# alexmillerdb/two_tower_recommender_model

Hardware: AMD Instinct MI355X
Metric: training pairs/sec at batch 8192 (per GPU) (higher is better)
Workload: dtype fp32; 1 GPU; northstar: 100M items x 50M users, emb_dim 128, towers [128, 64], single-hot uniform ids; global_batch=8192, per_gpu_batch=8192, emb_dim=128, tower_dtype=bf16 (MFMA, fp32 acc), parallelism=single-gpu hipgraph

## Files before the change

### two_tower_recommender_model_amd/csrc/tower.hip

```cpp
#include <vector>

#include "tt_common.h"
#include "dedup.h"
#include "shard.h"

namespace tt {

typedef __attribute__((ext_vector_type(8))) __bf16 bf16x8;
typedef __attribute__((ext_vector_type(4))) float f32x4;
typedef __attribute__((ext_vector_type(4))) __bf16 bf16x4;

constexpr int TR = 32;
constexpr int MAXW = 128;
constexpr int XCH = 128;
constexpr int LSTR = MAXW + 8;
constexpr int FSTR = MAXW + 4;
constexpr int MAXL = 4;

__device__ __forceinline__ int64_t strip_at(int64_t f, int64_t m, int64_t nf) {
  return (((m >> 5) * nf + f) << 5) + (m & 31);
}

struct TowerArgs {
  tt_tower_shape_t s;
// ... 1028 lines not shown
__host__ __device__ __forceinline__ int rk_swz(int row) {
  return (row & 3) | (((row & 1) | (((row >> 3) & 1) << 1)) << 2);
}
__host__ __device__ __forceinline__ int rk_off(int row, int col) {
  return row * 256 + (((col >> 3) ^ rk_swz(row)) << 4) + ((col & 7) << 1);
}
__device__ __forceinline__ int rk_perm(int mt, int rho) {
  return 32 * (mt >> 1) + 8 * (rho >> 2) + 4 * (mt & 1) + (rho & 3);
}
__device__ __forceinline__ bf16x8 rk_afwd(const char* img, int mt, int s, int rho, int q) {
  return *reinterpret_cast<const bf16x8*>(img + rk_off(rk_perm(mt, rho), 32 * s + 8 * q));
}
__device__ __forceinline__ bf16x8 rk_abwd(const char* img, int mt, int s, int lane) {
  const int q = lane >> 4, qq = (lane >> 2) & 3, p = lane & 3;
  const int row = 32 * s + 8 * q + qq;
  const int col = 32 * (mt >> 1) + 8 * p + 4 * (mt & 1);
  const bf16x4 lo = __builtin_amdgcn_ds_read_tr16_b64_v4bf16((lds_bf16x4*)(img + rk_off(row, col)));
  const bf16x4 hi = __builtin_amdgcn_ds_read_tr16_b64_v4bf16((lds_bf16x4*)(img + rk_off(row + 4, col)));
  return __builtin_shufflevector(lo, hi, 0, 1, 2, 3, 4, 5, 6, 7);
}
__device__ __forceinline__ bf16x8 rk_pack(const f32x4& a, const f32x4& b) {
  bf16x8 v;
#pragma unroll
  for (int j = 0; j < 4; ++j) {
    v[j] = (__bf16)a[j];
    v[4 + j] = (__bf16)b[j];
  }
  return v;
}
template <int MT, int S, bool BWD>
__device__ __forceinline__ void rk_gemm(f32x4 (&acc)[8], const char* img, const bf16x8 (&b)[4], int lane) {
  const int n = lane & 15, q = lane >> 4;
  bf16x8 fa[2][MT];
#pragma unroll
  for (int mt = 0; mt < MT; ++mt) {
    acc[mt] = (f32x4)(0.f);
    fa[0][mt] = BWD ? rk_abwd(img, mt, 0, lane) : rk_afwd(img, mt, 0, n, q);
  }
#pragma unroll
  for (int s = 0; s < S; ++s) {
    if (s + 1 < S) {
#pragma unroll
      for (int mt = 0; mt < MT; ++mt)
        fa[(s + 1) & 1][mt] = BWD ? rk_abwd(img, mt, s + 1, lane) : rk_afwd(img, mt, s + 1, n, q);
    }
    __builtin_amdgcn_sched_barrier(0);
#pragma unroll
    for (int mt = 0; mt < MT; ++mt)
      acc[mt] = __builtin_amdgcn_mfma_f32_16x16x32_bf16(fa[s & 1][mt], b[s], acc[mt], 0, 0, 0);
    __builtin_amdgcn_sched_barrier(0);
  }
}
template <int X>
__device__ __forceinline__ float rk_xor(float v) {
  if constexpr (X == 1) return dpp_f<0xB1>(v);
  if constexpr (X == 2) return dpp_f<0x4E>(v);
  if constexpr (X == 4) return dpp_f<0x1B>(dpp_f<0x141>(v));
  return dpp_f<0x128>(v);
}
template <int X, int H>
__device__ __forceinline__ void rk_halve(float* v, int n) {
  const bool up = (n & X) != 0;
#pragma unroll
  for (int i = 0; i < H; ++i) {
    const float keep = up ? v[H + i] : v[i], send = up ? v[i] : v[H + i];
    v[i] = keep + rk_xor<X>(send);
  }
}
template <int NV>
__device__ __forceinline__ void rk_colsum(float (&v)[NV], int n) {
  static_assert(NV == 32 || NV == 16, "column sum of 32 or 16 values per lane");
  rk_halve<8, NV / 2>(v, n);
  rk_halve<4, NV / 4>(v, n);
  rk_halve<2, NV / 8>(v, n);
  rk_halve<1, NV / 16>(v, n);
}
template <int NS>
__device__ __forceinline__ void rk_strip(const bf16x8 (&v)[4], __bf16* row, int q) {
#pragma unroll
  for (int s = 0; s < NS; ++s) *reinterpret_cast<bf16x8*>(row + 32 * s + 8 * q) = v[s];
}


__device__ __forceinline__ char* px_row(const tt_peer_direct_t& x, int64_t row, int64_t row_bytes) {
  char* base = reinterpret_cast<char*>(x.row0[0]);
  int64_t f0 = 0;
#pragma unroll
  for (int q = 1; q < TT_PEER_MAXW; ++q) {
    if (q < x.W && row >= x.first_row[q]) {
      base = reinterpret_cast<char*>(x.row0[q]);
      f0 = x.first_row[q];
    }
  }
  return base + (row - f0) * row_bytes;
}
__device__ __forceinline__ bool px_copy_unit(const tt_peer_direct_t& x, int64_t u, const uint4*& src, uint4*& dst) {
  int64_t pre = 0;
  bool hit = false;
#pragma unroll
  for (int q = 0; q < TT_PEER_MAXW; ++q) {
    const int64_t n = q < x.W ? x.copy_len[q] >> 4 : 0;
    if (!hit && u >= pre && u < pre + n) {
      src = reinterpret_cast<const uint4*>(x.copy_src[q]) + (u - pre);
      dst = reinterpret_cast<uint4*>(x.copy_dst[q]) + (u - pre);
      hit = true;
    }
    pre += n;
  }
  return hit;
}
__device__ __forceinline__ int64_t px_copy_units(const tt_peer_direct_t& x) {
  int64_t n = 0;
#pragma unroll
  for (int q = 0; q < TT_PEER_MAXW; ++q) n += q < x.W ? x.copy_len[q] >> 4 : 0;
  return n;
}

struct RkRaw {
  uint32_t lo, hi;
};
__device__ __forceinline__ RkRaw rk_raw(const void* p, bool wide, int64_t i) {
  RkRaw r;
  if (wide) {
    const uint2 v = reinterpret_cast<const uint2*>(p)[i];
    r.lo = v.x;
    r.hi = v.y;
  } else {
    r.lo = reinterpret_cast<const uint32_t*>(p)[i];
    r.hi = 0u;
  }
  return r;
}
__device__ __forceinline__ int64_t rk_id(RkRaw r, bool wide) {
  return wide ? (int64_t)(((uint64_t)r.hi << 32) | r.lo) : (int64_t)(int32_t)r.lo;
}
__device__ __forceinline__ float rk_label(RkRaw r, int dt) {
  if (dt == TT_I32) return (float)(int32_t)r.lo;
  if (dt == TT_I64) return (float)(int64_t)(((uint64_t)r.hi << 32) | r.lo);
  return __uint_as_float(r.lo);
}
#if TT_EXPERIMENTS
#define RK_STAMP(k) \
  do { if (a.stamps && lane == 0) a.stamps[8192 + ((int64_t)blockIdx.x * 16 + (k)) * 9 + wid] = (int64_t)__builtin_amdgcn_s_memrealtime(); } while (0)
#define RK_STAMP2(k) \
  do { if (a.stamps && lane == 0) a.stamps[8192 + ((int64_t)blockIdx.x * 16 + (k)) * 9 + 4 + wid] = (int64_t)__builtin_amdgcn_s_memrealtime(); } while (0)
#define RK_STAMP_IMG(k) \
  do { if (a.stamps && lane == 0) a.stamps[8192 + ((int64_t)blockIdx.x * 16 + (k)) * 9 + 8] = (int64_t)__builtin_amdgcn_s_memrealtime(); } while (0)
#else
#define RK_STAMP(k) do { } while (0)
#define RK_STAMP2(k) do { } while (0)
#define RK_STAMP_IMG(k) do { } while (0)
#endif

struct UpdateArgs {
  float* params;
  float* exp_avg;
  float* exp_avg_sq;
  const float* slab;
  const float* dbpart;
  int64_t P;
  int S;
  int nwg;
  int nseg;
  int64_t seg_off[2 * 2 * MAXL + 1];
  int32_t seg_t[2 * 2 * MAXL], seg_l[2 * 2 * MAXL], seg_isw[2 * 2 * MAXL], seg_n[2 * 2 * MAXL], seg_k[2 * 2 * MAXL];
  int64_t seg_wc[2 * 2 * MAXL];
  __bf16* wb;
  __bf16* wtb;
  __bf16* wbf;
  __bf16* wtbf;
  int skip_plain;
  float lr, beta1, beta2, eps, wd;
  int64_t* step_state;
  int do_adam;
  float* grads_out;
  const float* grads_in;
  const float* adam_pre;
  int out_copies;
  int64_t out_stride;
  int64_t out_off[16];
  float out_scale;
  int in_srcs;
  int64_t in_stride;
  char* wimg;
  PxWait wt;
#if TT_EXPERIMENTS
  int64_t* stamps;
#endif
};
#if TT_EXPERIMENTS
#define T3_STAMP(k) \
  do { if (a.stamps && threadIdx.x == 0 && bid < 512) a.stamps[(int64_t)bid * 4 + (k)] = (int64_t)__builtin_amdgcn_s_memrealtime(); } while (0)
#else
#define T3_STAMP(k) do { } while (0)
#endif

struct T3Seg {
  int64_t soff = 0, swc = 0;
  int sisw = 0, sk = 1, sn = 1, st_ = 0, sl_ = 0;
};
__device__ __forceinline__ T3Seg t3_seg(const UpdateArgs& a, int64_t i) {
  T3Seg g;
#pragma unroll
  for (int q = 0; q < 2 * 2 * MAXL; ++q) {
    if (q < a.nseg && i >= a.seg_off[q]) {
      g.soff = a.seg_off[q];
      g.sisw = a.seg_isw[q];
      g.sk = a.seg_k[q];
      g.sn = a.seg_n[q];
      g.swc = a.seg_wc[q];
      g.st_ = a.seg_t[q];
      g.sl_ = a.seg_l[q];
    }
  }
  return g;
}

__device__ __forceinline__ void t3_apply(const UpdateArgs& a, int64_t i, const T3Seg& sg, float p, float m,
                                         float v0, float g, float step_size, float bc2_sqrt, bool adam) {
#pragma clang fp contract(off)
  const int64_t e = i - sg.soff;
  if (a.grads_out) {
    if (a.out_copies <= 1) {
      a.grads_out[i] = g;
    } else {
      const float gs = g * a.out_scale;
      for (int q = 0; q < a.out_copies; ++q) a.grads_out[a.out_off[q] + i] = gs;
    }
  }
  if (adam) {
    if (a.wd != 0.f) g = g + a.wd * p;
    m = m + (1.f - a.beta1) * (g - m);
    const float v = v0 * a.beta2 + (1.f - a.beta2) * g * g;
    const float denom = sqrtf(v) / bc2_sqrt + a.eps;
    p = p + (-step_size) * m / denom;
    a.exp_avg[i] = m;
    a.exp_avg_sq[i] = v;
    a.params[i] = p;
  }
  if (sg.sisw) {
    const int K = sg.sk, N = sg.sn;
    const int64_t n = e / K, k = e - n * K;
    if (!a.skip_plain) {
      a.wb[sg.swc + e] = (__bf16)p;
      a.wtb[sg.swc + k * N + n] = (__bf16)p;
    }
    a.wbf[sg.swc + frag_off((int)n, (int)k, K)] = (__bf16)p;
    a.wtbf[sg.swc + frag_off((int)k, (int)n, N)] = (__bf16)p;
    if (a.wimg)
      *reinterpret_cast<__bf16*>(a.wimg + sg.st_ * RK_IMG_T + sg.sl_ * (RK_W0 * 256) + rk_off((int)n, (int)k)) = (__bf16)p;
  }
}

template <bool UPD, bool IDX, int IN, bool POOL = false>
__device__ __forceinline__ void tower_rows_body(const TowerArgs& a) {
  static_assert(IN == 128 || IN == 64, "row-owned T1: inputs of 128 or 64");
  static_assert(!POOL || (!UPD && !IDX), "pooled input: the plain T1 only");
  constexpr int NI = IN / 32;
  constexpr int MTI = IN / 16;
  __shared__ __attribute__((aligned(16))) char wimg[RK_IMG];
  __shared__ __attribute__((aligned(16))) float xo[2][2][16 * 64];
  __shared__ float bsum[2][RK_W0 + RK_W1];
  __shared__ float lrow[TR];
  __shared__ __attribute__((aligned(16))) float xr[4][16 * IN];
  const int lane = threadIdx.x & 63, wid = __builtin_amdgcn_readfirstlane(threadIdx.x >> 6);
  typedef __attribute__((address_space(3))) void lds_void;
  typedef __attribute__((address_space(1))) void glb_void;
  if (wid == 4) {
    RK_STAMP_IMG(0);
    if (!TDBG(16)) {
#pragma unroll
      for (int k = 0; k < RK_IMG / 1024; ++k)
        __builtin_amdgcn_global_load_lds((glb_void*)(a.wimg + k * 1024 + lane * 16), (lds_void*)(wimg + k * 1024), 16, 0, 0);
    }
    RK_STAMP_IMG(1);
    __builtin_amdgcn_s_waitcnt(0x0F70);
    RK_STAMP_IMG(2);
    __syncthreads();
    RK_STAMP_IMG(3);
    __syncthreads();
    __syncthreads();
    return;
  }
  const int t = wid >> 1, h = wid & 1, q = lane >> 4, n = lane & 15;
  const int tile = xcd_remap((int)blockIdx.x, (int)gridDim.x);
  const int64_t B = a.B, m0 = (int64_t)tile * TR, m = m0 + 16 * h + n;
  const bool live = m < B;
  RK_STAMP(0);
  const bool wide = a.gid_dtype == TT_I64;
  const int64_t mc = live ? m : 0;
  RkRaw id_raw{0u, 0u}, pout_raw{0u, 0u};
  if (IDX) {
    id_raw.lo = (uint32_t)(t ? a.gpos[1] : a.gpos[0])[mc];
    pout_raw.lo = a.gpos_out[0] ? (uint32_t)(t ? a.gpos_out[1] : a.gpos_out[0])[mc] : id_raw.lo;
  } else if (!POOL) {
    id_raw = rk_raw(t ? a.gcol[1] : a.gcol[0], wide, mc);
  }
  int32_t cl = -1;
  if (UPD) cl = a.dd.claim[live ? t * B + m : 0];
  const RkRaw lab_raw = rk_raw(a.labels, a.label_dtype == TT_I64, mc);
  f32x4 b0v[8], b1v[4];
  auto load_biases = [&]() {
    const float* b0p = a.params + a.boff[t][0];
    const float* b1p = a.params + a.boff[t][1];
#pragma unroll
    for (int mt = 0; mt < 8; ++mt) b0v[mt] = *reinterpret_cast<const f32x4*>(b0p + 32 * (mt >> 1) + 8 * q + 4 * (mt & 1));
#pragma unroll
    for (int mt = 0; mt < 4; ++mt) b1v[mt] = *reinterpret_cast<const f32x4*>(b1p + 32 * (mt >> 1) + 8 * q + 4 * (mt & 1));
  };
  load_biases();
  __builtin_amdgcn_sched_barrier(0);
  uint4 cpv = make_uint4(0u, 0u, 0u, 0u);
  uint4* cpd = nullptr;
  int64_t cp_per = 0, cp_end = 0;
  if constexpr (IDX) {
    if (a.xd.W) {
      const int64_t tot = px_copy_units(a.xd);
      cp_per = (tot + gridDim.x - 1) / gridDim.x;
      cp_end = min(tot, ((int64_t)blockIdx.x + 1) * cp_per);
      const int64_t u = (int64_t)blockIdx.x * cp_per + threadIdx.x;
      const uint4* cps;
      if (u < cp_end && px_copy_unit(a.xd, u, cps, cpd)) cpv = *cps;
      else cpd = nullptr;
    }
  }
  int64_t r;
  if (POOL) {
    r = live ? m : -1;
  } else if (IDX) {
    r = live ? (int64_t)(int32_t)id_raw.lo : -1;
  } else {
    const int64_t id = live ? rk_id(id_raw, wide) : 0;
    r = id != 0 ? py_mod64(id, t ? a.gmod[1] : a.gmod[0]) : -1;
  }
  const float* tab = POOL ? a.pooled + a.s.in_col[t] : (t ? a.gtab[1] : a.gtab[0]);
  const int64_t rstride = POOL ? a.ldp : IN;
  float* xw = xr[wid];
  constexpr int CPR = IDX ? IN / 8 : IN / 4;
  constexpr int RPI = 64 / CPR;
  if (IDX) {
    const int rr0 = lane / CPR, pc = lane % CPR;
    const char* src0 = reinterpret_cast<const char*>(t ? a.gsrc[1] : a.gsrc[0]);
#pragma unroll
    for (int i = 0; i < 16 / RPI; ++i) {
      const int row = RPI * i + rr0;
      const int64_t rid = __shfl((long long)r, row, 64);
      const char* src = src0 + (rid >= 0 ? rid : 0) * (IN * 2) + 16 * (pc ^ (row & (CPR - 1)));
      __builtin_amdgcn_global_load_lds((glb_void*)src, (lds_void*)(reinterpret_cast<char*>(xw) + i * 1024), 16, 0, 0);
    }
  } else {
    const int rr0 = lane / CPR, pc = lane % CPR;
#pragma unroll
    for (int i = 0; i < 16 / RPI; ++i) {
      const int row = RPI * i + rr0;
      const int64_t rid = __shfl((long long)r, row, 64);
      const float* src = tab + (rid >= 0 ? rid : 0) * rstride + 4 * (pc ^ row);
      if (!TDBG(32))
        __builtin_amdgcn_global_load_lds((glb_void*)src, (lds_void*)(xw + i * 256), 16, 0, 0);
    }
  }
  __builtin_amdgcn_sched_barrier(0);
  DdPend pend;
  pend.key = DD_EMPTY;
  const int32_t li = (int32_t)(t * B + m);
  if (!UPD && a.dd_on && q == 0 && live) {
    const uint64_t key = r >= 0 ? (((uint64_t)(t ? a.dd_table[1] : a.dd_table[0]) << DD_TABLE_SHIFT) | (uint64_t)r)
                                : DD_EMPTY;
// ... 689 lines not shown
  }
  for (; m + 32 <= me; m += 32) {
    const int64_t o = m + q * 8;
    const bf16x8 fa0 = *reinterpret_cast<const bf16x8*>(z0 + zo(o));
    const bf16x8 fa1 = *reinterpret_cast<const bf16x8*>(z1 + zo(o));
    const bf16x8 fb0 = *reinterpret_cast<const bf16x8*>(a0 + ao(o));
    const bf16x8 fb1 = *reinterpret_cast<const bf16x8*>(a1 + ao(o));
    acc[0][0] = __builtin_amdgcn_mfma_f32_16x16x32_bf16(fa0, fb0, acc[0][0], 0, 0, 0);
    acc[0][1] = __builtin_amdgcn_mfma_f32_16x16x32_bf16(fa0, fb1, acc[0][1], 0, 0, 0);
    acc[1][0] = __builtin_amdgcn_mfma_f32_16x16x32_bf16(fa1, fb0, acc[1][0], 0, 0, 0);
    acc[1][1] = __builtin_amdgcn_mfma_f32_16x16x32_bf16(fa1, fb1, acc[1][1], 0, 0, 0);
  }
  if (m < me) {
    bf16x8 fa0, fa1, fb0, fb1;
    for (int j = 0; j < 8; ++j) {
      const int64_t mm = m + q * 8 + j;
      const bool ok = mm < me;
      fa0[j] = ok ? z0[zo(mm)] : (__bf16)0.f;
      fa1[j] = ok ? z1[zo(mm)] : (__bf16)0.f;
      fb0[j] = ok ? a0[ao(mm)] : (__bf16)0.f;
      fb1[j] = ok ? a1[ao(mm)] : (__bf16)0.f;
    }
    acc[0][0] = __builtin_amdgcn_mfma_f32_16x16x32_bf16(fa0, fb0, acc[0][0], 0, 0, 0);
    acc[0][1] = __builtin_amdgcn_mfma_f32_16x16x32_bf16(fa0, fb1, acc[0][1], 0, 0, 0);
    acc[1][0] = __builtin_amdgcn_mfma_f32_16x16x32_bf16(fa1, fb0, acc[1][0], 0, 0, 0);
    acc[1][1] = __builtin_amdgcn_mfma_f32_16x16x32_bf16(fa1, fb1, acc[1][1], 0, 0, 0);
  }
  if (wid > 0) {
#pragma unroll
    for (int i = 0; i < 2; ++i)
#pragma unroll
      for (int j = 0; j < 2; ++j)
#pragma unroll
        for (int rr = 0; rr < 4; ++rr) red[wid - 1][((i * 2 + j) * 4 + rr) * 64 + lane] = acc[i][j][rr];
  }
  __syncthreads();
  if (wid > 0) return;
#pragma unroll
  for (int w = 0; w < 3; ++w)
#pragma unroll
    for (int i = 0; i < 2; ++i)
#pragma unroll
      for (int j = 0; j < 2; ++j)
#pragma unroll
        for (int rr = 0; rr < 4; ++rr) acc[i][j][rr] += red[w][((i * 2 + j) * 4 + rr) * 64 + lane];
  const int K = a.K[tl.t][tl.l];
  float* dst = a.slab + (int64_t)s * a.P + a.woff[tl.t][tl.l];
  for (int i = 0; i < 2; ++i)
    for (int j = 0; j < 2; ++j)
      for (int rr = 0; rr < 4; ++rr) {
        const int n = tl.n0 + i * 16 + q * 4 + rr;
        const int k = tl.k0 + j * 16 + r;
        dst[(int64_t)n * K + k] = acc[i][j][rr];
      }
}

__global__ void __launch_bounds__(256) tower_wgrad_kernel(WgradArgs a, const WgradTile* __restrict__ tiles) {
  __shared__ __attribute__((aligned(16))) char smem[T2_SMEM];
  if ((int)blockIdx.x < a.n_res)
    dd_resolve_block(a.dd, (int)blockIdx.x, a.n_res);
  else
    wgrad_block(a, tiles, (int)blockIdx.x - a.n_res, smem);
}

__global__ void __launch_bounds__(256) tower_wgrad_dedup_kernel(WgradArgs a, const WgradTile* __restrict__ tiles,
                                                                DdUpdateArgs d, int n_t2) {
  __shared__ __attribute__((aligned(16))) char smem[T2_SMEM];
  if ((int)blockIdx.x < n_t2)
    wgrad_block(a, tiles, (int)blockIdx.x, smem);
  else
    dd_update_block(d, (int)blockIdx.x - n_t2, smem);
}

struct InsertArgs {
  const void* col[2];
  int64_t mod[2];
  int32_t tab[2];
  int id_dtype;
  int64_t B;
  DedupWs dd;
  int xcd_wpt;
};
__device__ __forceinline__ int64_t ins_lookup(const InsertArgs& ins, int blk, int tid) {
  if (ins.xcd_wpt <= 0) return (int64_t)blk * 256 + tid;
  const int c = blk & 7, j = blk >> 3;
  const int t = j / ins.xcd_wpt, qi = j - t * ins.xcd_wpt;
  const int64_t b = (int64_t)c * (ins.B / 256) + 8 * qi + (tid >> 5);
  return (int64_t)t * ins.B + 32 * b + (tid & 31);
}

__device__ __forceinline__ void insert_next_block(const InsertArgs& ins, int blk) {
  const int lane = threadIdx.x & 63;
  const int64_t grp = (int64_t)blk * 4 + (threadIdx.x >> 6);
  const int64_t i = grp * 64 + lane;
  DdPend p;
  p.key = DD_EMPTY;
  if (i < 2 * ins.B) {
    const int t = i >= ins.B;
    const int64_t m = i - (t ? ins.B : 0);
    const int64_t id = load_id(t ? ins.col[1] : ins.col[0], ins.id_dtype, m);
    const uint64_t key = id != 0 ? (((uint64_t)(t ? ins.tab[1] : ins.tab[0]) << DD_TABLE_SHIFT) |
                                    (uint64_t)py_mod64(id, t ? ins.mod[1] : ins.mod[0]))
                                 : DD_EMPTY;
    dd_insert_begin(ins.dd, key, (int32_t)i, p);
  }
  if (grp < ins.dd.ovf_groups) dd_insert_defer_finish(ins.dd, p, (int32_t)(i < 2 * ins.B ? i : 0), (int)grp);
}

#if TT_EXPERIMENTS
#define RING_STAMP(p, k) \
  do { if ((p) && threadIdx.x == 0 && blockIdx.x < 2048) (p)[(int64_t)blockIdx.x * 2 + (k)] = (int64_t)__builtin_amdgcn_s_memrealtime(); } while (0)
#else
#define RING_STAMP(p, k) do { (void)(p); } while (0)
#endif

__global__ void __launch_bounds__(256) tower_wgrad_insert_kernel(WgradArgs a, const WgradTile* __restrict__ tiles,
                                                                 InsertArgs ins, int n_t2, int64_t* stamps) {
  __shared__ __attribute__((aligned(16))) char smem[T2_SMEM];
  RING_STAMP(stamps, 0);
  if ((int)blockIdx.x < n_t2)
    wgrad_block(a, tiles, (int)blockIdx.x, smem);
  else
    insert_next_block(ins, (int)blockIdx.x - n_t2);
  RING_STAMP(stamps, 1);
}

__global__ void __launch_bounds__(256, 3) tower_wgrad_route_rowwise_kernel(WgradArgs a, const WgradTile* __restrict__ tiles,
                                                                        RouteArgs r, DdUpdateArgs d, int n_t2,
                                                                        int n_cnt, int n_dd, PxWait w) {
  __shared__ __attribute__((aligned(16))) char smem[T2_SMEM];
  int b = (int)blockIdx.x;
  if (w.W) {
    if (b == 0) px_signal(w);
    if (b == 0 || (n_dd > 0 ? b < n_dd : b >= n_t2 + n_cnt)) px_wait(w);
  }
  if (n_dd > 0) {
    if (b < n_dd) {
      dd_update_block(d, b, smem);
      return;
    }
    b -= n_dd;
    if (b >= n_t2 + n_cnt) return;
  }
  if (b < n_t2) {
    wgrad_block(a, tiles, b, smem);
  } else if (b < n_t2 + n_cnt) {
    const int j = b - n_t2;
    route_count_block(r, j % r.nblk, j / r.nblk, reinterpret_cast<int (*)[RT_MAXW]>(smem));
  } else {
    dd_update_block(d, b - n_t2 - n_cnt, smem);
  }
}

__device__ __forceinline__ void update_block(const UpdateArgs& a, int bid, int nblocks) {
  T3_STAMP(0);
  if (a.wt.W) {
    if (bid == 0) px_signal(a.wt);
    px_wait(a.wt);
  }
  const int64_t i = (int64_t)bid * blockDim.x + threadIdx.x;
  int64_t t_step = 0;
  float step_size = 0.f, bc2_sqrt = 1.f;
  if (a.do_adam && a.adam_pre) {
    step_size = a.adam_pre[0];
    bc2_sqrt = a.adam_pre[1];
  } else if (a.do_adam) {
    t_step = a.step_state[0] + 1;
    const double bc1 = 1.0 - pow((double)a.beta1, (double)t_step);
    const double bc2 = 1.0 - pow((double)a.beta2, (double)t_step);
    step_size = (float)((double)a.lr / bc1);
    bc2_sqrt = (float)sqrt(bc2);
  }
  if (i < a.P) {
    const T3Seg sg = t3_seg(a, i);
    const float p = a.params[i];
    const float m = a.do_adam ? a.exp_avg[i] : 0.f, v = a.do_adam ? a.exp_avg_sq[i] : 0.f;
    float g = 0.f;
    if (a.grads_in) {
      g = a.grads_in[i];
      for (int q = 1; q < a.in_srcs; ++q) g += a.grads_in[(int64_t)q * a.in_stride + i];
    } else if (a.do_adam || a.grads_out) {
      if (sg.sisw) {
        for (int s0 = 0; s0 < a.S; s0 += 32) {
          float v[32];
#pragma unroll
          for (int u = 0; u < 32; ++u) {
            v[u] = s0 + u < a.S ? a.slab[(int64_t)(s0 + u) * a.P + i] : 0.f;
          }
#pragma unroll
          for (int u = 0; u < 32; ++u)
            if (s0 + u < a.S) g += v[u];
        }
      } else {
        g = a.slab[i];
      }
    }
    T3_STAMP(1);
    t3_apply(a, i, sg, p, m, v, g, step_size, bc2_sqrt, a.do_adam);
    T3_STAMP(2);
  }
  if (a.do_adam && !a.adam_pre) {
    __syncthreads();
    if (threadIdx.x == 0) {
      unsigned* counter = reinterpret_cast<unsigned*>(a.step_state + 1);
      const unsigned prev = __hip_atomic_fetch_add(counter, 1u, __ATOMIC_RELAXED, __HIP_MEMORY_SCOPE_AGENT);
      if (prev == (unsigned)nblocks - 1) {
        __hip_atomic_store(counter, 0u, __ATOMIC_RELAXED, __HIP_MEMORY_SCOPE_AGENT);
        __hip_atomic_store(reinterpret_cast<unsigned long long*>(a.step_state), (unsigned long long)t_step,
                           __ATOMIC_RELAXED, __HIP_MEMORY_SCOPE_AGENT);
      }
    }
  }
}

__global__ void __launch_bounds__(256) tower_update_kernel(UpdateArgs a) {
  update_block(a, xcd_remap((int)blockIdx.x, (int)gridDim.x), (int)gridDim.x);
}

__global__ void __launch_bounds__(256) tower_grads_place_gather_kernel(UpdateArgs a, RouteArgs r, GatherSegArgs g,
                                                                       int n_upd, int n_place) {
  __shared__ int base[RT_MAXW];
  __shared__ int wc[RT_BLOCK / 64][RT_MAXW];
  const int b = (int)blockIdx.x;
  if (g.epoch && b == 0 && threadIdx.x == 0)
    __hip_atomic_fetch_add(g.epoch, 1, __ATOMIC_RELAXED, __HIP_MEMORY_SCOPE_AGENT);
  if (b < n_upd) {
    update_block(a, xcd_remap(b, n_upd), n_upd);
  } else if (b < n_upd + n_place) {
    const int j = b - n_upd;
    route_place_block<true>(r, j % r.nblk, j / r.nblk, base, wc);
  } else {
    shard_gather_block(g, b - n_upd - n_place);
  }
}

constexpr int K3_RES_WGS = 32;
__global__ void __launch_bounds__(256) tower_update_dedup_resolve_kernel(UpdateArgs a, DdUpdateArgs d, DedupWs next,
                                                                         int n_dd, int64_t* stamps) {
  __shared__ __attribute__((aligned(16))) char smem[DD_SMEM];
  const int bid = (int)blockIdx.x;
  RING_STAMP(stamps, 0);
  if (bid < K3_RES_WGS)
    dd_resolve_block(next, bid, K3_RES_WGS);
  else if (bid < K3_RES_WGS + n_dd)
    dd_update_block(d, bid - K3_RES_WGS, smem);
  else
    update_block(a, bid - K3_RES_WGS - n_dd, (int)gridDim.x - K3_RES_WGS - n_dd);
  RING_STAMP(stamps, 1);
}

#ifndef TT_INS_PT
#define TT_INS_PT 1
#endif
constexpr int INS_PT = TT_INS_PT;
constexpr int INS_HS = 1024;
static_assert(INS_HS * (8 + 3 * 4) <= T2_SMEM, "the insert role's LDS hash fits the tail's LDS");
__device__ __forceinline__ void insert_next_full_block(const InsertArgs& ins, int blk, char* smem) {
  unsigned long long* hk = reinterpret_cast<unsigned long long*>(smem);
  int* hc = reinterpret_cast<int*>(smem + 8 * INS_HS);
  int* hb = hc + INS_HS;
  int* hg = hb + INS_HS;
  const DedupWs& ws = ins.dd;
  for (int q = threadIdx.x; q < INS_HS; q += 256) {
    hk[q] = DD_EMPTY;
    hc[q] = 0;
  }
  int64_t iv[INS_PT];
  uint64_t key[INS_PT];
#pragma unroll
  for (int u = 0; u < INS_PT; ++u) {
    const int64_t i = INS_PT == 1 ? ins_lookup(ins, blk, (int)threadIdx.x)
                                  : ((int64_t)blk * INS_PT + u) * 256 + threadIdx.x;
    iv[u] = i;
    key[u] = DD_EMPTY;
    if (i < 2 * ins.B) {
      const int t = i >= ins.B;
      const int64_t m = i - (t ? ins.B : 0);
      const int64_t id = load_id(t ? ins.col[1] : ins.col[0], ins.id_dtype, m);
      if (id != 0)
        key[u] = ((uint64_t)(t ? ins.tab[1] : ins.tab[0]) << DD_TABLE_SHIFT) |
                 (uint64_t)py_mod64(id, t ? ins.mod[1] : ins.mod[0]);
      ws.lkey[i] = key[u];
    }
  }
  __syncthreads();
  int hl[INS_PT], rank[INS_PT];
#pragma unroll
  for (int u = 0; u < INS_PT; ++u) {
    hl[u] = -1;
    rank[u] = 0;
    if (key[u] != DD_EMPTY) {
      unsigned h = (unsigned)dd_mix64(key[u]) & (INS_HS - 1);
      while (true) {
        const unsigned long long prev = atomicCAS(&hk[h], (unsigned long long)DD_EMPTY, (unsigned long long)key[u]);
        if (prev == DD_EMPTY || prev == key[u]) break;
        h = (h + 1) & (INS_HS - 1);
      }
      hl[u] = (int)h;
      rank[u] = atomicAdd(&hc[h], 1);
    }
  }
  __syncthreads();
  const uint64_t mask = (uint64_t)ws.cap - 1;
#pragma unroll
  for (int u = 0; u < INS_PT; ++u) {
    if (hl[u] >= 0 && rank[u] == 0) {
      const uint64_t c = (uint64_t)hc[hl[u]];
      uint64_t g = dd_mix64(key[u]) & mask;
      int base;
      while (true) {
        unsigned long long* w = reinterpret_cast<unsigned long long*>(&ws.slots[g].word);
        const unsigned long long prev =
            atomicCAS(w, (unsigned long long)DD_EMPTY, (unsigned long long)((key[u] << DD_CNT_BITS) | c));
        if (prev == DD_EMPTY) {
          base = 0;
          break;
        }
        if ((prev >> DD_CNT_BITS) == key[u]) {
          base = (int)(atomicAdd(w, (unsigned long long)c) & DD_CNT_MASK);
          break;
        }
        g = (g + 1) & mask;
      }
      hb[hl[u]] = base;
      hg[hl[u]] = (int)g;
    }
  }
  __syncthreads();
#pragma unroll
  for (int u = 0; u < INS_PT; ++u) {
    const int64_t i = iv[u];
    if (i >= 2 * ins.B) continue;
    if (hl[u] < 0) {
      ws.claim[i] = -1;
      continue;
    }
    const int k = hb[hl[u]] + rank[u], h = hg[hl[u]];
    ws.claim[i] = k == 0 ? h : -1;
    if (k < DD_INL) {
      ws.slots[h].item[k] = (int32_t)i;
    } else if (k == DD_INL) {
      const int q = atomicAdd(&ws.ctr[0], 1);
      if (q < ws.hot_cap) {
        ws.hot[q] = h;
        ws.hkey[q] = key[u];
      }
    }
  }
}

template <bool LIST>
__global__ void __launch_bounds__(256, 3) tower_tail_kernel(WgradArgs a2, const WgradTile* __restrict__ tiles,
                                                         InsertArgs ins, DdUpdateArgs d, int n_ins, int n_t2,
                                                         int64_t* stamps) {
  __shared__ __attribute__((aligned(16))) char smem[T2_SMEM];
  int b = (int)blockIdx.x;
  RING_STAMP(stamps, 0);
  if (b < n_ins)
    insert_next_full_block(ins, b, smem);
  else if ((b -= n_ins) < n_t2)
    wgrad_block(a2, tiles, b, smem);
  else
    dd_update_block<LIST>(d, b - n_t2, smem);
  RING_STAMP(stamps, 1);
}

__global__ void __launch_bounds__(256) tower_update_dedup_kernel(UpdateArgs a, DdUpdateArgs d, int n_dd) {
  __shared__ __attribute__((aligned(16))) char smem[DD_SMEM];
  if ((int)blockIdx.x < n_dd)
    dd_update_block(d, (int)blockIdx.x, smem);
  else
    update_block(a, (int)blockIdx.x - n_dd, (int)gridDim.x - n_dd);
}


struct TowerLayout {
  int64_t P;
  int64_t PW;
  int64_t woff[2][MAXL], boff[2][MAXL], wcoff[2][MAXL];
  int32_t K[2][MAXL];
// ... 397 lines not shown
  a.pooled_out = pooled_out;
  if (dedup_ws) {
    if (!dedup_tables) return fail(TT_EINVAL, "tower_gather: dedup needs the key table of each tower");
    if (int rc = check_dedup_ws(dedup_ws, dedup_ws_bytes, dedup_max_lookups, 2 * B, "tower_gather", true)) return rc;
    for (int t = 0; t < 2; ++t) {
      if (dedup_tables[t] < 0 || dedup_tables[t] >= TT_MAX_TABLES || num_embeddings[t] >= (1ll << DD_TABLE_SHIFT))
        return fail(TT_EINVAL, "tower_gather: bad dedup table");
      a.dd_table[t] = dedup_tables[t];
    }
    dedup_layout(dedup_ws, dedup_max_lookups, &a.dd);
    a.dd_on = 1;
  }
  return launch_t1(shape, B, a, nullptr, ldp, gpooled,
                   {params, labels, label_dtype, grad_scale, logits, workspace, ws_bytes, stream});
}

int tt_tower_fwd_bwd_kjt(const tt_tower_shape_t* shape, int64_t B, const void* values, int id_dtype,
                         const int32_t* offsets, const int64_t* num_rows, const float* const* table_rows,
                         float* pooled_out, int64_t ldp, float* gpooled, const float* params, const void* labels,
                         int label_dtype, float grad_scale, float* logits, void* workspace, size_t ws_bytes,
                         void* stream) {
  if (!values || !offsets || !num_rows || !table_rows) return fail(TT_EINVAL, "tower_fwd_bwd_kjt: null pointer");
  if (id_dtype != TT_I32 && id_dtype != TT_I64) return fail(TT_EINVAL, "tower_fwd_bwd_kjt: ids must be int32/int64");
  TowerArgs a{};
  for (int t = 0; t < 2; ++t) {
    if (!table_rows[t] || num_rows[t] < 1) return fail(TT_EINVAL, "tower_fwd_bwd_kjt: bad table");
    if (reinterpret_cast<uintptr_t>(table_rows[t]) & 15)
      return fail(TT_EINVAL, "tower_fwd_bwd_kjt: rows not 16-B aligned");
    a.gtab[t] = table_rows[t];
    a.gmod[t] = num_rows[t];
    a.moff[t] = offsets + (int64_t)t * B;
  }
  a.mval = values;
  a.gid_dtype = id_dtype;
  a.pooled_out = pooled_out;
  return launch_t1(shape, B, a, nullptr, ldp, gpooled,
                   {params, labels, label_dtype, grad_scale, logits, workspace, ws_bytes, stream});
}

static int tower_indexed(const tt_tower_shape_t* shape, int64_t B, const int32_t* const* pos,
                         const float* const* rows_in, float* const* grad_rows_out, const T1Common& c, int bf16_rows) {
  if (!pos || !rows_in || !grad_rows_out) return fail(TT_EINVAL, "tower_indexed: null pointer");
  TowerArgs a{};
  a.gsrc_bf16 = bf16_rows;
  for (int t = 0; t < 2; ++t) {
    if (!pos[t] || !rows_in[t] || !grad_rows_out[t]) return fail(TT_EINVAL, "tower_indexed: null pointer");
    if ((reinterpret_cast<uintptr_t>(rows_in[t]) & 15) || (reinterpret_cast<uintptr_t>(grad_rows_out[t]) & 15))
      return fail(TT_EINVAL, "tower_indexed: rows not 16-B aligned");
    a.gpos[t] = pos[t];
    a.gsrc[t] = rows_in[t];
    a.gdst[t] = grad_rows_out[t];
  }
  return launch_t1(shape, B, a, nullptr,
                   std::max(shape->in_col[0] + shape->in_dim[0], shape->in_col[1] + shape->in_dim[1]), nullptr, c);
}

int tt_tower_fwd_bwd_indexed(const tt_tower_shape_t* shape, int64_t B, const int32_t* const* pos,
                             const float* const* rows_in, float* const* grad_rows_out, const float* params,
                             const void* labels, int label_dtype, float grad_scale, float* logits, void* workspace,
                             size_t ws_bytes, void* stream) {
  return tower_indexed(shape, B, pos, rows_in, grad_rows_out,
                       {params, labels, label_dtype, grad_scale, logits, workspace, ws_bytes, stream}, 0);
}

int tt_tower_fwd_bwd_indexed_bf16(const tt_tower_shape_t* shape, int64_t B, const int32_t* const* pos,
                                  const void* const* rows_in, float* const* grad_rows_out, const float* params,
                                  const void* labels, int label_dtype, float grad_scale, float* logits,
                                  void* workspace, size_t ws_bytes, void* stream) {
  return tower_indexed(shape, B, pos, reinterpret_cast<const float* const*>(rows_in), grad_rows_out,
                       {params, labels, label_dtype, grad_scale, logits, workspace, ws_bytes, stream}, 1);
}

int tt_tower_wgrad(const tt_tower_shape_t* shape, int64_t B, float* loss, void* workspace, size_t ws_bytes,
                   void* stream) {
  tt_wgrad_role_t w{};
  w.loss = loss;
  WgradArgs a{};
  int64_t wgs = 0;
  TowerLayout L;
  int rc = wgrad_args(shape, B, workspace, ws_bytes, w, a, &wgs, L);
  if (rc) return rc;
  tower_wgrad_kernel<<<dim3((unsigned)wgs), dim3(256), 0, as_stream(stream)>>>(a, wgrad_tiles(workspace, a));
  return check_launch("tower_wgrad");
}

int tt_tower_wgrad_pre(const tt_tower_shape_t* shape, int64_t B, float* loss, void* workspace, size_t ws_bytes,
                       int64_t* adam_step_state, float adam_lr, float adam_beta1, float adam_beta2, void* dedup_ws,
                       size_t dedup_ws_bytes, int64_t dedup_max_lookups, void* stream) {
  if (!adam_step_state) return fail(TT_EINVAL, "tower_wgrad_pre: null Adam step state");
  const tt_wgrad_role_t w{loss, adam_step_state, adam_lr, adam_beta1, adam_beta2};
  WgradArgs a{};
  int64_t wgs = 0;
  TowerLayout L;
  int rc = wgrad_args(shape, B, workspace, ws_bytes, w, a, &wgs, L);
  if (rc) return rc;
  if (dedup_ws) {
    if ((rc = check_dedup_ws(dedup_ws, dedup_ws_bytes, dedup_max_lookups, 1, "tower_wgrad_pre", true))) return rc;
    dedup_layout(dedup_ws, dedup_max_lookups, &a.dd);
    a.n_res = 64;
    wgs += a.n_res;
  }
  tower_wgrad_kernel<<<dim3((unsigned)wgs), dim3(256), 0, as_stream(stream)>>>(a, wgrad_tiles(workspace, a));
  return check_launch("tower_wgrad_pre");
}

static int fused_wgrad_adagrad(const tt_launch_plan_t& p, void* stream) {
  WgradArgs a{};
  int64_t wgs = 0;
  TowerLayout L;
  int rc = wgrad_args(p.shape, p.B, p.workspace, p.ws_bytes, p.wgrad, a, &wgs, L);
  if (rc) return rc;
  DdUpdateArgs d{};
  int64_t dd_grid = 0;
  if ((rc = dedup_update_args(p.adagrad, d, &dd_grid))) return rc;
  if (wgs + dd_grid > INT32_MAX) return fail(TT_EINVAL, "tower_wgrad_rowwise_adagrad: grid too large");
  tower_wgrad_dedup_kernel<<<dim3((unsigned)(wgs + dd_grid)), dim3(256), 0, as_stream(stream)>>>(
      a, wgrad_tiles(p.workspace, a), d, (int)wgs);
  return check_launch("tower_wgrad_rowwise_adagrad");
}

struct T3Opts {
  int64_t* step_state = nullptr;
  float lr = 0.f;
  int do_adam = 0;
  const float* grads_in = nullptr;
  int in_srcs = 1;
  int64_t in_stride = 0;
  bool adam_pre = false;
  const DdUpdateArgs* dd = nullptr;
  int64_t dd_grid = 0;
  const tt_peer_wait_t* wait = nullptr;
};

static int replicated_check(const tt_update_role_t& u) {
  if (!u.base || !u.offsets || u.copies < 1 || u.copies > 16) return fail(TT_EINVAL, "tower_grads_replicated: bad output");
  return TT_OK;
}

static int t3_args(const tt_tower_shape_t* shape, int64_t B, void* workspace, size_t ws_bytes,
                   const tt_update_role_t& u, const T3Opts& o, UpdateArgs& a, int64_t* grid, TowerLayout& L) {
  int rc = tower_ws_layout(shape, B, workspace, ws_bytes, &L);
  if (rc) return rc;
  const bool rep = u.replicated != 0;
  if (!u.params || (o.do_adam && (!u.exp_avg || !u.exp_avg_sq || (!o.step_state && !o.adam_pre))))
    return fail(TT_EINVAL, "tower: null pointer");
  if (rep && u.copies > 16) return fail(TT_EINVAL, "tower: at most 16 gradient copies");
  char* ws = reinterpret_cast<char*>(workspace);
  a = UpdateArgs{};
  a.params = u.params;
  a.exp_avg = rep ? nullptr : u.exp_avg;
  a.exp_avg_sq = rep ? nullptr : u.exp_avg_sq;
  a.slab = reinterpret_cast<const float*>(ws + L.o_slab);
  a.dbpart = reinterpret_cast<const float*>(ws + L.o_dbpart);
  a.P = L.P;
  a.S = L.S;
  a.nwg = L.nwg;
  int sg = 0;
  for (int t = 0; t < 2; ++t)
    for (int l = 0; l < shape->L; ++l) {
      a.seg_off[sg] = L.woff[t][l];
      a.seg_t[sg] = t; a.seg_l[sg] = l; a.seg_isw[sg] = 1;
      a.seg_n[sg] = shape->width[l]; a.seg_k[sg] = L.K[t][l];
      a.seg_wc[sg] = L.wcoff[t][l];
      ++sg;
      a.seg_off[sg] = L.boff[t][l];
      a.seg_t[sg] = t; a.seg_l[sg] = l; a.seg_isw[sg] = 0;
      a.seg_n[sg] = shape->width[l]; a.seg_k[sg] = 1;
      a.seg_wc[sg] = 0;
      ++sg;
    }
  a.nseg = sg;
  a.seg_off[sg] = L.P;
  a.wb = reinterpret_cast<__bf16*>(ws + L.o_wb);
  a.wtb = reinterpret_cast<__bf16*>(ws + L.o_wtb);
  a.wbf = reinterpret_cast<__bf16*>(ws + L.o_wbf);
  a.wtbf = reinterpret_cast<__bf16*>(ws + L.o_wtbf);
  a.wimg = L.rows ? ws + L.o_wimg : nullptr;
  a.skip_plain = shape->L == 2 && shape->in_dim[0] <= 128 && shape->in_dim[1] <= 128 &&
                 !(shape->flags & TT_TOWER_GENERAL_T1);
  a.lr = o.lr;
  a.beta1 = rep ? 0.9f : u.beta1; a.beta2 = rep ? 0.999f : u.beta2; a.eps = rep ? 1e-8f : u.eps;
  a.wd = rep ? 0.f : u.weight_decay;
  a.step_state = o.step_state;
  a.do_adam = o.do_adam;
  a.grads_out = rep ? u.base : u.grads_out;
  a.grads_in = o.grads_in;
  a.adam_pre = o.adam_pre ? reinterpret_cast<const float*>(ws + L.o_counter) : nullptr;
  a.out_copies = !rep ? 1 : u.copies == 1 ? 2 : u.copies;
  for (int q = 0; rep && u.offsets && q < a.out_copies; ++q) a.out_off[q] = u.offsets[q < u.copies ? q : 0];
  a.out_scale = rep ? u.scale : 1.f;
  a.in_srcs = o.in_srcs;
  a.in_stride = o.in_stride;
  *grid = ceil_div(L.P, 256);
  return TT_OK;
}

static int launch_t3(const tt_tower_shape_t* shape, int64_t B, void* workspace, size_t ws_bytes,
                     const tt_update_role_t& u, const T3Opts& o, void* stream) {
  UpdateArgs a;
  int64_t g3 = 0;
  TowerLayout L;
  int rc = t3_args(shape, B, workspace, ws_bytes, u, o, a, &g3, L);
  if (rc) return rc;
  if ((rc = peer_wait_args(o.wait, a.wt, "tower_update"))) return rc;
  if (o.dd) {
    if (o.dd_grid + g3 > INT32_MAX) return fail(TT_EINVAL, "tower_update_rowwise_adagrad: grid too large");
    tower_update_dedup_kernel<<<dim3((unsigned)(o.dd_grid + g3)), dim3(256), 0, as_stream(stream)>>>(a, *o.dd,
                                                                                                      (int)o.dd_grid);
    return check_launch("tower_update_rowwise_adagrad");
  }
#if TT_EXPERIMENTS
  if (getenv("TT_RING_STAMPS"))
    a.stamps = reinterpret_cast<int64_t*>(reinterpret_cast<char*>(workspace) + L.o_dbg) + 6144;
#endif
  int bs = 256;
#if TT_EXPERIMENTS
  if (const char* e = getenv("TT_T3_BLOCK")) bs = atoi(e) == 128 ? 128 : 256;
#endif
  tower_update_kernel<<<dim3((unsigned)ceil_div(a.P, (int64_t)bs)), dim3(bs), 0, as_stream(stream)>>>(a);
  return check_launch("tower_update");
}

static tt_update_role_t adam_role(float* params, float* exp_avg, float* exp_avg_sq, float eps, float beta1,
                                  float beta2, float weight_decay, float* grads_out) {
  tt_update_role_t u{};
  u.params = params, u.exp_avg = exp_avg, u.exp_avg_sq = exp_avg_sq;
  u.eps = eps, u.beta1 = beta1, u.beta2 = beta2, u.weight_decay = weight_decay, u.grads_out = grads_out;
  return u;
}

int tt_tower_update(const tt_tower_shape_t* shape, int64_t B, float* params, float* exp_avg, float* exp_avg_sq,
                    float lr, float beta1, float beta2, float eps, float weight_decay, int64_t* step_state,
                    int do_adam, float* grads_out, void* workspace, size_t ws_bytes, void* stream) {
  return launch_t3(shape, B, workspace, ws_bytes,
                   adam_role(params, exp_avg, exp_avg_sq, eps, beta1, beta2, weight_decay, grads_out),
                   {.step_state = step_state, .lr = lr, .do_adam = do_adam}, stream);
}

int tt_tower_update_pre(const tt_tower_shape_t* shape, int64_t B, float* params, float* exp_avg, float* exp_avg_sq,
                        float eps, float beta1, float beta2, float weight_decay, float* grads_out, void* workspace,
                        size_t ws_bytes, void* stream) {
  return launch_t3(shape, B, workspace, ws_bytes,
                   adam_role(params, exp_avg, exp_avg_sq, eps, beta1, beta2, weight_decay, grads_out),
                   {.do_adam = 1, .adam_pre = true}, stream);
}

static int fused_update_adagrad(const tt_launch_plan_t& p, void* stream) {
  TowerLayout L;
  int rc = tower_ws_layout(p.shape, p.B, p.workspace, p.ws_bytes, &L);
  if (rc) return rc;
  DdUpdateArgs d{};
  int64_t dd_grid = 0;
  if ((rc = dedup_update_args(p.adagrad, d, &dd_grid))) return rc;
  return launch_t3(p.shape, p.B, p.workspace, p.ws_bytes, p.update,
                   {.do_adam = 1, .adam_pre = true, .dd = &d, .dd_grid = dd_grid}, stream);
}

int tt_tower_adam_grads(const tt_tower_shape_t* shape, int64_t B, float* params, const float* grads,
                        float* exp_avg, float* exp_avg_sq, float lr, float beta1, float beta2, float eps,
                        float weight_decay, int64_t* step_state, void* workspace, size_t ws_bytes, void* stream) {
  if (!grads) return fail(TT_EINVAL, "tower_adam_grads: null gradient");
  return launch_t3(shape, B, workspace, ws_bytes,
                   adam_role(params, exp_avg, exp_avg_sq, eps, beta1, beta2, weight_decay, nullptr),
                   {.step_state = step_state, .lr = lr, .do_adam = 1, .grads_in = grads}, stream);
}

int tt_tower_grads_replicated(const tt_tower_shape_t* shape, int64_t B, float* params, float* base, int copies,
                              const int64_t* offsets, float scale, void* workspace, size_t ws_bytes, void* stream) {
  tt_update_role_t u{};
  u.params = params, u.replicated = 1, u.copies = copies, u.base = base, u.offsets = offsets, u.scale = scale;
  if (int rc = replicated_check(u)) return rc;
  for (int q = 0; q < copies; ++q)
    if (offsets[q] < 0) return fail(TT_EINVAL, "tower_grads_replicated: negative offset");
  return launch_t3(shape, B, workspace, ws_bytes, u, {}, stream);
}

int tt_tower_adam_pre_grads_sum(const tt_tower_shape_t* shape, int64_t B, float* params, const float* grads, int nsrc,
                                int64_t src_stride, float* exp_avg, float* exp_avg_sq, float eps, float beta1,
                                float beta2, float weight_decay, void* workspace, size_t ws_bytes,
                                const tt_peer_wait_t* wait, void* stream) {
  TowerLayout L;
  int rc = tower_ws_layout(shape, B, workspace, ws_bytes, &L);
  if (rc) return rc;
  if (!grads || nsrc < 1 || (nsrc > 1 && src_stride < L.P)) return fail(TT_EINVAL, "tower_adam_pre_grads_sum: bad gradient");
  if (wait && wait->W != nsrc) return fail(TT_EINVAL, "tower_adam_pre_grads_sum: wait.W must be nsrc");
  return launch_t3(shape, B, workspace, ws_bytes,
                   adam_role(params, exp_avg, exp_avg_sq, eps, beta1, beta2, weight_decay, nullptr),
                   {.do_adam = 1, .grads_in = grads, .in_srcs = nsrc, .in_stride = src_stride, .adam_pre = true,
                    .wait = wait},
                   stream);
}

}

namespace tt {
static int fused_route_args(const tt_launch_plan_t& p, RouteArgs& r) {
  if (p.B < 1) return fail(TT_EINVAL, "route: bad batch / segment capacity");
  return route_args(p.route, p.B, RT_SEGS, "route", r);
}
}

extern "C" {

static int fused_wgrad_route_count_adagrad(const tt_launch_plan_t& p, void* stream) {
  if (!p.wgrad.adam_step_state) return fail(TT_EINVAL, "tower_wgrad_route_rowwise: null Adam step state");
  PxWait pw;
  if (int rc = peer_wait_args(p.wait, pw, "tower_wgrad_route_rowwise")) return rc;
  WgradArgs a{};
  int64_t wgs = 0;
  TowerLayout L;
  int rc = wgrad_args(p.shape, p.B, p.workspace, p.ws_bytes, p.wgrad, a, &wgs, L);
  if (rc) return rc;
  RouteArgs r{};
  if ((rc = fused_route_args(p, r))) return rc;
  DdUpdateArgs d{};
  int64_t dd_grid = 0;
  if ((rc = dedup_update_args(p.adagrad, d, &dd_grid))) return rc;
  const int64_t n_cnt = (int64_t)r.nblk * r.F;
  if (wgs + n_cnt + dd_grid > INT32_MAX) return fail(TT_EINVAL, "tower_wgrad_route_rowwise: grid too large");
  d.xcd = d.hot_wgs % 8 == 0 ? 1 : 0;
#if TT_EXPERIMENTS
  static const bool dd_first = !getenv("TT_U_DD_FIRST") || atoi(getenv("TT_U_DD_FIRST")) != 0;
#else
  constexpr bool dd_first = true;
#endif
// ... 270 lines not shown
```

Measured before the change: 275.0 million pairs/s.

## Pack tower update segment table and issue slab loads before segment lookup

Repacks the per-segment table in the update kernel args into 16-byte records of 32-bit fields, places the hot fields at the front of a 64-byte-aligned struct, and keeps them in scalar registers so segment lookup needs fewer kernarg loads. The update block now issues the first batch of slab gradient loads and the param/Adam state loads before resolving the segment. It then sums slab partials unconditionally with clamped indices and selects the bias value afterwards, so memory latency overlaps with the lookup. It also narrows P to 32 bits and adds a host check, which limits the supported parameter count, and issues redundant slab reads for bias segments.

```diff
diff --git a/two_tower_recommender_model_amd/csrc/tower.hip b/two_tower_recommender_model_amd/csrc/tower.hip
--- a/two_tower_recommender_model_amd/csrc/tower.hip
+++ b/two_tower_recommender_model_amd/csrc/tower.hip
@@ -1204,19 +1204,23 @@
 #define RK_STAMP_IMG(k) do { } while (0)
 #endif
 
-struct UpdateArgs {
+typedef uint32_t t3_u32x4 __attribute__((ext_vector_type(4)));
+constexpr int T3_NSEG = 2 * 2 * MAXL;
+
+struct alignas(64) UpdateArgs {
   float* params;
   float* exp_avg;
   float* exp_avg_sq;
   const float* slab;
+  const float* adam_pre;
+  const float* grads_in;
+  int32_t P;
+  int S;
+  int do_adam;
+  int nseg;
+  t3_u32x4 seg[T3_NSEG];
   const float* dbpart;
-  int64_t P;
-  int S;
   int nwg;
-  int nseg;
-  int64_t seg_off[2 * 2 * MAXL + 1];
-  int32_t seg_t[2 * 2 * MAXL], seg_l[2 * 2 * MAXL], seg_isw[2 * 2 * MAXL], seg_n[2 * 2 * MAXL], seg_k[2 * 2 * MAXL];
-  int64_t seg_wc[2 * 2 * MAXL];
   __bf16* wb;
   __bf16* wtb;
   __bf16* wbf;
@@ -1224,10 +1228,7 @@
   int skip_plain;
   float lr, beta1, beta2, eps, wd;
   int64_t* step_state;
-  int do_adam;
   float* grads_out;
-  const float* grads_in;
-  const float* adam_pre;
   int out_copies;
   int64_t out_stride;
   int64_t out_off[16];
@@ -1241,6 +1242,11 @@
 #endif
 };
 #if TT_EXPERIMENTS
+#define T3_BLOCK ((int)blockDim.x)
+#else
+#define T3_BLOCK 256
+#endif
+#if TT_EXPERIMENTS
 #define T3_STAMP(k) \
   do { if (a.stamps && threadIdx.x == 0 && bid < 512) a.stamps[(int64_t)bid * 4 + (k)] = (int64_t)__builtin_amdgcn_s_memrealtime(); } while (0)
 #else
@@ -1251,20 +1257,34 @@
   int64_t soff = 0, swc = 0;
   int sisw = 0, sk = 1, sn = 1, st_ = 0, sl_ = 0;
 };
-__device__ __forceinline__ T3Seg t3_seg(const UpdateArgs& a, int64_t i) {
+__device__ __forceinline__ T3Seg t3_seg(const UpdateArgs& a, int64_t i, int nseg) {
+  const int32_t ii = (int32_t)i;
+  int32_t off = 0, wc = 0;
+  uint32_t nk = 1u | 1u << 16, meta = 0;
+  const auto half = [&](int q0) {
+    t3_u32x4 r[8];
+#pragma unroll
+    for (int q = 0; q < 8; ++q) r[q] = a.seg[q0 + q];
+    asm volatile("" ::"s"(r[0]), "s"(r[1]), "s"(r[2]), "s"(r[3]), "s"(r[4]), "s"(r[5]), "s"(r[6]), "s"(r[7]));
+#pragma unroll
+    for (int q = 0; q < 8; ++q) {
+      const bool c = ii >= (int32_t)r[q].x;
+      off = c ? (int32_t)r[q].x : off;
+      wc = c ? (int32_t)r[q].y : wc;
+      nk = c ? r[q].z : nk;
+      meta = c ? r[q].w : meta;
+    }
+  };
+  half(0);
+  if (nseg > 8) half(8);
   T3Seg g;
-#pragma unroll
-  for (int q = 0; q < 2 * 2 * MAXL; ++q) {
-    if (q < a.nseg && i >= a.seg_off[q]) {
-      g.soff = a.seg_off[q];
-      g.sisw = a.seg_isw[q];
-      g.sk = a.seg_k[q];
-      g.sn = a.seg_n[q];
-      g.swc = a.seg_wc[q];
-      g.st_ = a.seg_t[q];
-      g.sl_ = a.seg_l[q];
-    }
-  }
+  g.soff = off;
+  g.swc = wc;
+  g.sisw = (int)(meta & 1u);
+  g.st_ = (int)(meta >> 1 & 1u);
+  g.sl_ = (int)(meta >> 2);
+  g.sn = (int)(nk & 0xffffu);
+  g.sk = (int)(nk >> 16);
   return g;
 }
 
@@ -2260,54 +2280,82 @@
   }
 }
 
-__device__ __forceinline__ void update_block(const UpdateArgs& a, int bid, int nblocks) {
+template <bool REMAP = false>
+__device__ __forceinline__ void update_block(const UpdateArgs& a, int b, int nblocks) {
+  const float* params = a.params;
+  const float* exp_avg = a.exp_avg;
+  const float* exp_avg_sq = a.exp_avg_sq;
+  const float* slab = a.slab;
+  const float* adam_pre = a.adam_pre;
+  const float* grads_in = a.grads_in;
+  const float* grads_out = a.grads_out;
+  int64_t P = a.P;
+  int S = a.S, do_adam = a.do_adam, nseg = a.nseg, wt_w = a.wt.W;
+  asm volatile(""
+               : "+s"(P), "+s"(S), "+s"(do_adam), "+s"(nseg), "+s"(wt_w), "+s"(nblocks)
+               : "s"(slab), "s"(adam_pre), "s"(grads_in), "s"(params), "s"(exp_avg), "s"(exp_avg_sq), "s"(grads_out));
+  const int bid = REMAP ? xcd_remap(b, nblocks) : b;
   T3_STAMP(0);
-  if (a.wt.W) {
+  if (wt_w) {
     if (bid == 0) px_signal(a.wt);
     px_wait(a.wt);
   }
-  const int64_t i = (int64_t)bid * blockDim.x + threadIdx.x;
+  const int64_t i = (int64_t)bid * T3_BLOCK + threadIdx.x;
   int64_t t_step = 0;
   float step_size = 0.f, bc2_sqrt = 1.f;
-  if (a.do_adam && a.adam_pre) {
-    step_size = a.adam_pre[0];
-    bc2_sqrt = a.adam_pre[1];
-  } else if (a.do_adam) {
+  const bool pre = do_adam && adam_pre;
+  if (do_adam && !pre) {
     t_step = a.step_state[0] + 1;
     const double bc1 = 1.0 - pow((double)a.beta1, (double)t_step);
     const double bc2 = 1.0 - pow((double)a.beta2, (double)t_step);
     step_size = (float)((double)a.lr / bc1);
     bc2_sqrt = (float)sqrt(bc2);
   }
-  if (i < a.P) {
-    const T3Seg sg = t3_seg(a, i);
-    const float p = a.params[i];
-    const float m = a.do_adam ? a.exp_avg[i] : 0.f, v = a.do_adam ? a.exp_avg_sq[i] : 0.f;
-    float g = 0.f;
-    if (a.grads_in) {
-      g = a.grads_in[i];
-      for (int q = 1; q < a.in_srcs; ++q) g += a.grads_in[(int64_t)q * a.in_stride + i];
-    } else if (a.do_adam || a.grads_out) {
-      if (sg.sisw) {
-        for (int s0 = 0; s0 < a.S; s0 += 32) {
-          float v[32];
-#pragma unroll
-          for (int u = 0; u < 32; ++u) {
-            v[u] = s0 + u < a.S ? a.slab[(int64_t)(s0 + u) * a.P + i] : 0.f;
-          }
-#pragma unroll
-          for (int u = 0; u < 32; ++u)
-            if (s0 + u < a.S) g += v[u];
-        }
-      } else {
-        g = a.slab[i];
-      }
-    }
+  if (i < P) {
+    float sv[32];
+    const auto slab_issue = [&](int s0) {
+#pragma unroll
+      for (int u = 0; u < 32; ++u)
+        sv[u] = (slab + (uint32_t)(s0 + u < S ? s0 + u : S - 1) * (uint32_t)P)[(uint32_t)i];
+    };
+    const auto slab_sum = [&](int s0, float g) {
+#pragma unroll
+      for (int u = 0; u < 32; ++u) g = s0 + u < S ? g + sv[u] : g;
+      return g;
+    };
+    const float* const mp = do_adam ? exp_avg : params;
+    const float* const vp = do_adam ? exp_avg_sq : params;
+    const float* const sp = pre ? adam_pre : params;
+    float g = 0.f, p, m, v, pre0, pre1;
+    const auto state_issue = [&]() { p = params[i], m = mp[i], v = vp[i], pre0 = sp[0], pre1 = sp[1]; };
+    T3Seg sg;
+    if (!grads_in && (do_adam || grads_out)) {
+      slab_issue(0);
+      state_issue();
+      sg = t3_seg(a, i, nseg);
+      asm volatile("" : "+v"(sv[0]) : "v"(sg.soff), "v"(sg.swc), "v"(sg.sisw), "v"(sg.sk), "v"(sg.sn), "v"(sg.st_), "v"(sg.sl_));
+      const float gb = sv[0];
+      g = slab_sum(0, g);
+      for (int s0 = 32; s0 < S; s0 += 32) {
+        slab_issue(s0);
+        g = slab_sum(s0, g);
+      }
+      g = sg.sisw ? g : gb;
+    } else {
+      if (grads_in) {
+        g = grads_in[i];
+        for (int q = 1; q < a.in_srcs; ++q) g += grads_in[(int64_t)q * a.in_stride + i];
+      }
+      state_issue();
+      sg = t3_seg(a, i, nseg);
+    }
+    if (!do_adam) m = 0.f, v = 0.f;
+    if (pre) step_size = pre0, bc2_sqrt = pre1;
     T3_STAMP(1);
-    t3_apply(a, i, sg, p, m, v, g, step_size, bc2_sqrt, a.do_adam);
+    t3_apply(a, i, sg, p, m, v, g, step_size, bc2_sqrt, do_adam);
     T3_STAMP(2);
   }
-  if (a.do_adam && !a.adam_pre) {
+  if (do_adam && !pre) {
     __syncthreads();
     if (threadIdx.x == 0) {
       unsigned* counter = reinterpret_cast<unsigned*>(a.step_state + 1);
@@ -2322,7 +2370,7 @@
 }
 
 __global__ void __launch_bounds__(256) tower_update_kernel(UpdateArgs a) {
-  update_block(a, xcd_remap((int)blockIdx.x, (int)gridDim.x), (int)gridDim.x);
+  update_block<true>(a, (int)blockIdx.x, (int)gridDim.x);
 }
 
 __global__ void __launch_bounds__(256) tower_grads_place_gather_kernel(UpdateArgs a, RouteArgs r, GatherSegArgs g,
@@ -2333,7 +2381,7 @@
   if (g.epoch && b == 0 && threadIdx.x == 0)
     __hip_atomic_fetch_add(g.epoch, 1, __ATOMIC_RELAXED, __HIP_MEMORY_SCOPE_AGENT);
   if (b < n_upd) {
-    update_block(a, xcd_remap(b, n_upd), n_upd);
+    update_block<true>(a, b, n_upd);
   } else if (b < n_upd + n_place) {
     const int j = b - n_upd;
     route_place_block<true>(r, j % r.nblk, j / r.nblk, base, wc);
@@ -3037,25 +3085,23 @@
   a.exp_avg_sq = rep ? nullptr : u.exp_avg_sq;
   a.slab = reinterpret_cast<const float*>(ws + L.o_slab);
   a.dbpart = reinterpret_cast<const float*>(ws + L.o_dbpart);
-  a.P = L.P;
+  a.P = (int32_t)L.P;
   a.S = L.S;
   a.nwg = L.nwg;
+  if ((int64_t)L.S * L.P >= INT32_MAX / 4 || L.PW >= INT32_MAX)
+    return fail(TT_EINVAL, "tower: parameter vector too long for the segment table");
   int sg = 0;
+  const auto rec = [&](int64_t off, int64_t wc, int n, int k, int isw, int t, int l) {
+    a.seg[sg++] = t3_u32x4{(uint32_t)off, (uint32_t)wc, (uint32_t)n | (uint32_t)k << 16,
+                           (uint32_t)isw | (uint32_t)t << 1 | (uint32_t)l << 2};
+  };
   for (int t = 0; t < 2; ++t)
     for (int l = 0; l < shape->L; ++l) {
-      a.seg_off[sg] = L.woff[t][l];
-      a.seg_t[sg] = t; a.seg_l[sg] = l; a.seg_isw[sg] = 1;
-      a.seg_n[sg] = shape->width[l]; a.seg_k[sg] = L.K[t][l];
-      a.seg_wc[sg] = L.wcoff[t][l];
-      ++sg;
-      a.seg_off[sg] = L.boff[t][l];
-      a.seg_t[sg] = t; a.seg_l[sg] = l; a.seg_isw[sg] = 0;
-      a.seg_n[sg] = shape->width[l]; a.seg_k[sg] = 1;
-      a.seg_wc[sg] = 0;
-      ++sg;
+      rec(L.woff[t][l], L.wcoff[t][l], shape->width[l], L.K[t][l], 1, t, l);
+      rec(L.boff[t][l], 0, shape->width[l], 1, 0, t, l);
     }
   a.nseg = sg;
-  a.seg_off[sg] = L.P;
+  while (sg < T3_NSEG) rec(INT32_MAX, 0, 1, 1, 0, 0, 0);
   a.wb = reinterpret_cast<__bf16*>(ws + L.o_wb);
   a.wtb = reinterpret_cast<__bf16*>(ws + L.o_wtb);
   a.wbf = reinterpret_cast<__bf16*>(ws + L.o_wbf);
```

Measured after the change: 291.0 million pairs/s (median of 6 runs). 5.8% higher.
